# Kamino666/video_features

Hardware: NVIDIA H100
Metric: frames/sec CLIP-ViT-B/32 @224px (higher is better)
Workload: dtype f16

## Files before the change

video_features_b200/csrc/common.cuh:

```cuda
#pragma once
#include <cuda.h>
#include <cuda_runtime.h>
#include <cuda_fp16.h>
#include <stdint.h>

namespace vf {

__device__ __forceinline__ uint32_t smem_u32(const void* p) {
    return static_cast<uint32_t>(__cvta_generic_to_shared(p));
}

__device__ __forceinline__ void mbar_init(uint64_t* bar, uint32_t count) {
    asm volatile("mbarrier.init.shared::cta.b64 [%0], %1;" ::"r"(smem_u32(bar)), "r"(count));
}
__device__ __forceinline__ void fence_mbar_init() {
    asm volatile("fence.mbarrier_init.release.cluster;" ::: "memory");
}
__device__ __forceinline__ void mbar_expect_tx(uint64_t* bar, uint32_t bytes) {
    asm volatile("mbarrier.arrive.expect_tx.shared::cta.b64 _, [%0], %1;" ::"r"(smem_u32(bar)), "r"(bytes)
                 : "memory");
}
__device__ __forceinline__ void mbar_arrive(uint64_t* bar) {
    asm volatile("mbarrier.arrive.shared::cta.b64 _, [%0];" ::"r"(smem_u32(bar)) : "memory");
}
__device__ __forceinline__ void mbar_wait(uint64_t* bar, uint32_t parity) {
    asm volatile(
        "{\n"
        ".reg .pred P1;\n"
        "LAB_WAIT:\n"
        "mbarrier.try_wait.parity.shared::cta.b64 P1, [%0], %1;\n"
        "@P1 bra DONE;\n"
        "bra LAB_WAIT;\n"
        "DONE:\n"
        "}" ::"r"(smem_u32(bar)),
        "r"(parity)
        : "memory");
}

__device__ __forceinline__ void tma_prefetch_desc(const CUtensorMap* tm) {
    asm volatile("prefetch.tensormap [%0];" ::"l"(reinterpret_cast<uint64_t>(tm)) : "memory");
}
__device__ __forceinline__ void tma_load_2d(void* smem_dst, const CUtensorMap* tm, uint64_t* bar, int c0, int c1) {
    asm volatile(
        "cp.async.bulk.tensor.2d.shared::cluster.global.mbarrier::complete_tx::bytes [%0], [%1, {%3, %4}], [%2];" ::"r"(
            smem_u32(smem_dst)),
        "l"(reinterpret_cast<uint64_t>(tm)), "r"(smem_u32(bar)), "r"(c0), "r"(c1)
        : "memory");
}
__device__ __forceinline__ void tma_load_4d(void* smem_dst, const CUtensorMap* tm, uint64_t* bar, int c0, int c1,
                                            int c2, int c3) {
    asm volatile(
        "cp.async.bulk.tensor.4d.shared::cluster.global.mbarrier::complete_tx::bytes [%0], [%1, {%3, %4, %5, %6}], "
        "[%2];" ::"r"(smem_u32(smem_dst)),
        "l"(reinterpret_cast<uint64_t>(tm)), "r"(smem_u32(bar)), "r"(c0), "r"(c1), "r"(c2), "r"(c3)
        : "memory");
}
__device__ __forceinline__ void tma_load_5d(void* smem_dst, const CUtensorMap* tm, uint64_t* bar, int c0, int c1,
                                            int c2, int c3, int c4) {
    asm volatile(
        "cp.async.bulk.tensor.5d.shared::cluster.global.mbarrier::complete_tx::bytes [%0], [%1, {%3, %4, %5, %6, "
        "%7}], [%2];" ::"r"(smem_u32(smem_dst)),
        "l"(reinterpret_cast<uint64_t>(tm)), "r"(smem_u32(bar)), "r"(c0), "r"(c1), "r"(c2), "r"(c3), "r"(c4)
        : "memory");
}

__device__ __forceinline__ void tma_store_2d(const CUtensorMap* tm, const void* smem_src, int c0, int c1) {
    asm volatile("cp.async.bulk.tensor.2d.global.shared::cta.bulk_group [%0, {%2, %3}], [%1];" ::"l"(
                     reinterpret_cast<uint64_t>(tm)),
                 "r"(smem_u32(smem_src)), "r"(c0), "r"(c1)
                 : "memory");
}
__device__ __forceinline__ void tma_reduce_add_2d(const CUtensorMap* tm, const void* smem_src, int c0, int c1) {
    asm volatile("cp.reduce.async.bulk.tensor.2d.global.shared::cta.add.tile.bulk_group [%0, {%2, %3}], [%1];" ::"l"(
                     reinterpret_cast<uint64_t>(tm)),
                 "r"(smem_u32(smem_src)), "r"(c0), "r"(c1)
                 : "memory");
}
__device__ __forceinline__ void red_add_f32x4(float* gptr, float4 v) {
    asm volatile("red.global.add.v4.f32 [%0], {%1, %2, %3, %4};" ::"l"(gptr), "f"(v.x), "f"(v.y), "f"(v.z), "f"(v.w) : "memory");
}
__device__ __forceinline__ void bulk_commit() { asm volatile("cp.async.bulk.commit_group;" ::: "memory"); }
template <int N>
__device__ __forceinline__ void bulk_wait_read() {
    asm volatile("cp.async.bulk.wait_group.read %0;" ::"n"(N) : "memory");
}
template <int N>
__device__ __forceinline__ void bulk_wait() {
    asm volatile("cp.async.bulk.wait_group %0;" ::"n"(N) : "memory");
}
__device__ __forceinline__ void st_shared_b32(uint32_t addr, uint32_t v) {
    asm volatile("st.shared.b32 [%0], %1;" ::"r"(addr), "r"(v) : "memory");
}
__device__ __forceinline__ void st_shared_v2_f32(uint32_t addr, float x, float y) {
    asm volatile("st.shared.v2.f32 [%0], {%1, %2};" ::"r"(addr), "f"(x), "f"(y) : "memory");
}
__device__ __forceinline__ void fence_proxy_async() { asm volatile("fence.proxy.async.shared::cta;" ::: "memory"); }
__device__ __forceinline__ void named_bar_sync(uint32_t id, uint32_t nthreads) {
    asm volatile("bar.sync %0, %1;" ::"r"(id), "r"(nthreads) : "memory");
}
__device__ __forceinline__ void named_bar_arrive(uint32_t id, uint32_t nthreads) {
    asm volatile("bar.arrive %0, %1;" ::"r"(id), "r"(nthreads) : "memory");
}
template <uint32_t N>
__device__ __forceinline__ void setmaxnreg_dec() {
    asm volatile("setmaxnreg.dec.sync.aligned.u32 %0;" ::"n"(N));
}
template <uint32_t N>
__device__ __forceinline__ void setmaxnreg_inc() {
    asm volatile("setmaxnreg.inc.sync.aligned.u32 %0;" ::"n"(N));
}

__device__ __forceinline__ uint64_t wgmma_desc_sw128(const void* smem_tile) {
    uint64_t d = 0;
    d |= static_cast<uint64_t>((smem_u32(smem_tile) & 0x3FFFF) >> 4);
    d |= static_cast<uint64_t>(1) << 16;
    d |= static_cast<uint64_t>(1024 >> 4) << 32;
    d |= static_cast<uint64_t>(1) << 62;
    return d;
}
__device__ __forceinline__ void wgmma_fence() { asm volatile("wgmma.fence.sync.aligned;" ::: "memory"); }
__device__ __forceinline__ void wgmma_commit() { asm volatile("wgmma.commit_group.sync.aligned;" ::: "memory"); }
template <int N>
__device__ __forceinline__ void wgmma_wait() {
    asm volatile("wgmma.wait_group.sync.aligned %0;" ::"n"(N) : "memory");
}
template <int R>
__device__ __forceinline__ void wgmma_fence_regs(float* d) {
#pragma unroll
    for (int i = 0; i < R; ++i) asm volatile("" : "+f"(d[i])::"memory");
}

__device__ __forceinline__ float warp_sum(float v) {
#pragma unroll
    for (int o = 16; o > 0; o >>= 1) v += __shfl_xor_sync(0xffffffffu, v, o);
    return v;
}
__device__ __forceinline__ float warp_max(float v) {
#pragma unroll
    for (int o = 16; o > 0; o >>= 1) v = fmaxf(v, __shfl_xor_sync(0xffffffffu, v, o));
    return v;
}
__device__ __forceinline__ uint32_t pack_half2(float a, float b) {
    __half2 h = __floats2half2_rn(a, b);
    return *reinterpret_cast<uint32_t*>(&h);
}

}
```

video_features_b200/csrc/gemm.cu:

```cuda
#include "gemm_kernel.cuh"

namespace vf {

extern template int launch_bn<1, false, true>(GEMM_LAUNCH_ARGS);
extern template int launch_bn<1, true, true>(GEMM_LAUNCH_ARGS);
extern template int launch_bn<1, false, false>(GEMM_LAUNCH_ARGS);
extern template int launch_bn<1, true, false>(GEMM_LAUNCH_ARGS);
extern template int launch_bn<2, false, false>(GEMM_LAUNCH_ARGS);
extern template int launch_bn<2, true, false>(GEMM_LAUNCH_ARGS);

namespace {

typedef CUresult (*EncodeTiledFn)(CUtensorMap*, CUtensorMapDataType, cuuint32_t, void*, const cuuint64_t*,
                                  const cuuint64_t*, const cuuint32_t*, const cuuint32_t*, CUtensorMapInterleave,
                                  CUtensorMapSwizzle, CUtensorMapL2promotion, CUtensorMapFloatOOBfill);

EncodeTiledFn get_encode_tiled() {
    static EncodeTiledFn fn = nullptr;
    if (fn) return fn;
    void* p = nullptr;
    cudaDriverEntryPointQueryResult q;
    if (cudaGetDriverEntryPoint("cuTensorMapEncodeTiled", &p, cudaEnableDefault, &q) != cudaSuccess ||
        q != cudaDriverEntryPointSuccess)
        return nullptr;
    fn = reinterpret_cast<EncodeTiledFn>(p);
    return fn;
}

}

int device_sm_count() {
    static std::atomic<int> sms[64];
    int dev = 0;
    if (cudaGetDevice(&dev) != cudaSuccess || dev < 0 || dev >= 64) return 132;
    int v = sms[dev].load(std::memory_order_relaxed);
    if (v == 0) {
        if (cudaDeviceGetAttribute(&v, cudaDevAttrMultiProcessorCount, dev) != cudaSuccess || v <= 0) v = 132;
        sms[dev].store(v, std::memory_order_relaxed);
    }
    return v;
}

int make_tmap_2d(CUtensorMap* out, const void* base, int elem_bytes, uint64_t rows, uint64_t cols,
                 uint64_t row_pitch_bytes, uint32_t box_rows, uint32_t box_cols) {
    EncodeTiledFn enc = get_encode_tiled();
    if (!enc) return fail(VF_ERR_CUDA, "cuTensorMapEncodeTiled entry point unavailable (no CUDA driver?)");
    if ((reinterpret_cast<uintptr_t>(base) & 15) || (row_pitch_bytes & 15))
        return fail(VF_ERR_INVALID, "TMA operand must be 16-byte aligned with a 16-byte multiple row pitch");
    if (box_cols * uint32_t(elem_bytes) != 128) return fail(VF_ERR_INVALID, "TMA box rows must be 128 bytes");
    const CUtensorMapDataType dt = elem_bytes == 2 ? CU_TENSOR_MAP_DATA_TYPE_FLOAT16 : CU_TENSOR_MAP_DATA_TYPE_FLOAT32;
    cuuint64_t dims[2] = {cols, rows};
    cuuint64_t strides[1] = {row_pitch_bytes};
    cuuint32_t box[2] = {box_cols, box_rows};
    cuuint32_t estr[2] = {1, 1};
    CUresult r = enc(out, dt, 2, const_cast<void*>(base), dims, strides, box, estr, CU_TENSOR_MAP_INTERLEAVE_NONE,
                     CU_TENSOR_MAP_SWIZZLE_128B, CU_TENSOR_MAP_L2_PROMOTION_L2_256B, CU_TENSOR_MAP_FLOAT_OOB_FILL_NONE);
    if (r != CUDA_SUCCESS) return fail(VF_ERR_CUDA, "cuTensorMapEncodeTiled failed with CUresult %d", int(r));
    return VF_OK;
}

struct GemmProf {
    bool on = false;
    std::vector<cudaEvent_t> ev;
    size_t used = 0;
    double flops = 0.0;
};
static thread_local GemmProf g_prof;

template <bool PP>
static int run_gemm_launch(const CUtensorMap& tmA, const CUtensorMap& tmB, const CUtensorMap& tmD,
                           const CUtensorMap& tmD2, int bn, const GemmEpi& ep, int M, int N, const ConvGeom& cg,
                           cudaStream_t stream) {
    const bool split = ep.split_off > 0 && !ep.out_f32;
    if constexpr (!PP) {
        if (cg.nsplit == 2)
            return split ? launch_bn<2, true, PP>(tmA, tmB, tmD, tmD2, bn, ep, M, N, cg, stream)
                         : launch_bn<2, false, PP>(tmA, tmB, tmD, tmD2, bn, ep, M, N, cg, stream);
    }
    return split ? launch_bn<1, true, PP>(tmA, tmB, tmD, tmD2, bn, ep, M, N, cg, stream)
                 : launch_bn<1, false, PP>(tmA, tmB, tmD, tmD2, bn, ep, M, N, cg, stream);
}

static int run_gemm(const CUtensorMap& tmA, bool pp, const __half* B, int ldb, int64_t Ktot, int M, int N,
                    const ConvGeom& cg, const GemmEpi& ep, cudaStream_t stream) {
    if (!ep.out) return fail(VF_ERR_INVALID, "gemm: null output");
    if (reinterpret_cast<uintptr_t>(ep.out) & 15) return fail(VF_ERR_INVALID, "gemm: output must be 16-byte aligned");
    if (ep.accumulate && !ep.out_f32) return fail(VF_ERR_INVALID, "gemm: accumulate needs fp32 output");
    if (N % 8) return fail(VF_ERR_INVALID, "gemm: N=%d must be a multiple of 8", N);
    if (ep.act < VF_ACT_NONE || ep.act > VF_ACT_LEAKY) return fail(VF_ERR_INVALID, "gemm: unknown activation %d", ep.act);
    if (ep.out_f32 ? (ep.ldo % 4) : (ep.ldo % 8)) return fail(VF_ERR_INVALID, "gemm: ldo breaks 16-byte rows");
    if (ep.split_off && (ep.out_f32 || ep.split_off < N || ep.split_off % 8))
        return fail(VF_ERR_INVALID, "gemm: split output needs fp16 out and split_off >= N, multiple of 8");
    const int bm = tile_rows(pp);
    const int64_t num_m = (M + bm - 1) / bm, sms = device_sm_count();
    int bn = 256;
    int64_t best = INT64_MAX;
    for (int cand : {256, 192, 128, 64}) {
        const int64_t cost = (num_m * ((N + cand - 1) / cand) + sms - 1) / sms * cand;
        if (cost < best) { best = cost; bn = cand; }
    }
    CUtensorMap tmB, tmD, tmD2;
    VF_TRY(make_tmap_2d(&tmB, B, 2, uint64_t(N), uint64_t(Ktot), uint64_t(ldb) * 2, uint32_t(bn), BK));
    const int eb = ep.out_f32 ? 4 : 2;
    VF_TRY(make_tmap_2d(&tmD, ep.out, eb, uint64_t(M), uint64_t(N), uint64_t(ep.ldo) * eb, EPI_ROWS, 128 / eb));
    if (ep.split_off)
        VF_TRY(make_tmap_2d(&tmD2, static_cast<__half*>(ep.out) + ep.split_off, eb, uint64_t(M), uint64_t(N),
                            uint64_t(ep.ldo) * eb, EPI_ROWS, 128 / eb));
    else
        tmD2 = tmD;
    auto launch = [&] {
        return pp ? run_gemm_launch<true>(tmA, tmB, tmD, tmD2, bn, ep, M, N, cg, stream)
                  : run_gemm_launch<false>(tmA, tmB, tmD, tmD2, bn, ep, M, N, cg, stream);
    };
    if (!g_prof.on) return launch();
    if (g_prof.used + 2 > g_prof.ev.size())
        for (int i = 0; i < 2; ++i) {
            cudaEvent_t e;
            VF_CUDA(cudaEventCreate(&e));
            g_prof.ev.push_back(e);
        }
    VF_CUDA(cudaEventRecord(g_prof.ev[g_prof.used], stream));
    const int st = launch();
    VF_CUDA(cudaEventRecord(g_prof.ev[g_prof.used + 1], stream));
    g_prof.used += 2;
    double kexec = double(Ktot);
    if (cg.nsplit == 2 && cg.lo_mask) {
        const int kpt = (cg.k_per_tap + BK - 1) / BK;
        int skipped = 0;
        for (int kk = 0; kk < kpt && kk < 64; ++kk) skipped += int((cg.lo_mask >> kk) & 1ull);
        kexec -= double(cg.ntaps) * skipped * BK;
    }
    g_prof.flops += 2.0 * double(M) * double(N) * kexec;
    return st;
}

bool gemm_profile_on() { return g_prof.on; }
int gemm_profile(int enable) {
    g_prof.on = enable != 0;
    return VF_OK;
}
int gemm_profile_read(double* ms, int64_t* launches, double* flops) {
    VF_CUDA(cudaDeviceSynchronize());
    double t = 0.0;
    for (size_t i = 0; i + 1 < g_prof.used; i += 2) {
        float x = 0.f;
        VF_CUDA(cudaEventElapsedTime(&x, g_prof.ev[i], g_prof.ev[i + 1]));
        t += x;
    }
    if (ms) *ms = t;
    if (launches) *launches = int64_t(g_prof.used / 2);
    if (flops) *flops = g_prof.flops;
    g_prof.used = 0;
    g_prof.flops = 0.0;
    return VF_OK;
}

int gemm_f16(const __half* A, int lda, const __half* B, int ldb, int M, int N, int K, const GemmEpi& ep,
             cudaStream_t stream) {
    if (M <= 0 || N <= 0 || K <= 0) return fail(VF_ERR_INVALID, "gemm: empty problem %dx%dx%d", M, N, K);
    if (K % 8 || lda % 8 || ldb % 8) return fail(VF_ERR_INVALID, "gemm: K/lda/ldb must be multiples of 8");
    ConvGeom cg;
    memset(&cg, 0, sizeof(cg));
    cg.ntaps = 1;
    cg.k_per_tap = K;
    cg.nsplit = 1;
    CUtensorMap tmA;
    VF_TRY(make_tmap_2d(&tmA, A, 2, uint64_t(M), uint64_t(K), uint64_t(lda) * 2, tile_rows(true), BK));
    return run_gemm(tmA, true, B, ldb, K, M, N, cg, ep, stream);
}

int conv_gemm_f16(const __half* X, int C, int64_t P, const __half* Wt, int N, const ConvGeom& g, const GemmEpi& ep,
                  cudaStream_t stream) {
    if (P <= 0 || P > 0x7fffffff || N <= 0 || C <= 0) return fail(VF_ERR_INVALID, "conv_gemm: bad size");
    if (C % 8) return fail(VF_ERR_INVALID, "conv_gemm: C=%d must be a multiple of 8", C);
    if (g.ntaps < 1 || g.ntaps > 64 || g.k_per_tap < 8 || g.k_per_tap % 8)
        return fail(VF_ERR_INVALID, "conv_gemm: bad tap geometry (%d taps x %d)", g.ntaps, g.k_per_tap);
    if (g.nsplit != 1 && g.nsplit != 2) return fail(VF_ERR_INVALID, "conv_gemm: nsplit must be 1 or 2");
    const int kpt = (g.k_per_tap + BK - 1) / BK;
    if (g.lo_mask && (kpt > 64 || (kpt < 64 && (g.lo_mask >> kpt) != 0)))
        return fail(VF_ERR_INVALID, "conv_gemm: lo_mask 0x%llx names K blocks beyond the %d of a tap", g.lo_mask, kpt);
    if (g.mask && (g.Tp < 1 || g.Hp < 1 || g.Wp < 1 || g.row0 < 0))
        return fail(VF_ERR_INVALID, "conv_gemm: bad mask volume %dx%dx%d, row0 %d", g.Tp, g.Hp, g.Wp, g.row0);
    CUtensorMap tmA;
    VF_TRY(make_tmap_2d(&tmA, X, 2, uint64_t(P), uint64_t(g.k_per_tap), uint64_t(C) * 2, tile_rows(false), BK));
    const int64_t Ktot = int64_t(g.ntaps) * g.k_per_tap * g.nsplit;
    if (Ktot % 8) return fail(VF_ERR_INVALID, "conv_gemm: K must be a multiple of 8");
    return run_gemm(tmA, false, Wt, int(Ktot), Ktot, int(P), N, g, ep, stream);
}

}
```

video_features_b200/csrc/gemm_inst_pp.cu:

```cuda
#include "gemm_kernel.cuh"

namespace vf {
template int launch_bn<1, false, true>(GEMM_LAUNCH_ARGS);
template int launch_bn<1, true, true>(GEMM_LAUNCH_ARGS);
}
```

video_features_b200/csrc/gemm_kernel.cuh:

```cuda
#pragma once
#include <stdarg.h>
#include <stdlib.h>
#include <string.h>

#include <atomic>
#include <vector>

#include "common.cuh"
#include "internal.h"
#include "wgmma.cuh"

namespace vf {

namespace {

constexpr int BK = 64;
constexpr int THREADS = 384;
constexpr uint32_t PRODUCER_REGS = 40, CONSUMER_REGS = 232;
constexpr int EPI_ROWS = 64;
constexpr uint32_t STG_BYTES = EPI_ROWS * 128;
constexpr uint32_t STAGING_BYTES = 2 * 2 * STG_BYTES;
constexpr uint32_t SMEM_LIMIT = 227 * 1024;
constexpr uint32_t MAX_STAGES = 8;
constexpr uint32_t RING_BUDGET = SMEM_LIMIT - STAGING_BYTES - 2 * MAX_STAGES * 8 - 1024;

template <int BN, int NSPLIT, bool PP>
struct GemmCfg {
    static constexpr int BM = PP ? 64 : 128;
    static constexpr uint32_t A_BYTES = BM * BK * 2;
    static constexpr uint32_t B_TILE = BN * BK * 2;
    static constexpr uint32_t B_BYTES = NSPLIT * B_TILE;
    static constexpr uint32_t STAGE_BYTES = A_BYTES + B_BYTES;
    static constexpr int STAGES = RING_BUDGET / STAGE_BYTES > MAX_STAGES ? MAX_STAGES : int(RING_BUDGET / STAGE_BYTES);
    static constexpr uint32_t BAR_BYTES = 2 * STAGES * 8;
    static constexpr uint32_t SMEM_BYTES = STAGES * STAGE_BYTES + STAGING_BYTES + BAR_BYTES + 1024;
    static_assert(STAGES >= 2, "at least two pipeline stages");
    static_assert(SMEM_BYTES <= SMEM_LIMIT, "shared memory budget");
    static_assert(A_BYTES % 1024 == 0 && B_TILE % 1024 == 0, "swizzle-128B tiles must stay 1024-byte aligned");
};

constexpr int tile_rows(bool pp) { return pp ? GemmCfg<64, 1, true>::BM : GemmCfg<64, 1, false>::BM; }

template <int ACT>
__device__ __forceinline__ float apply_act(float v) {
    if (ACT == VF_ACT_QUICKGELU) {
        return __fdividef(v, 1.0f + __expf(-1.702f * v));
    } else if (ACT == VF_ACT_RELU) {
        return fmaxf(v, 0.0f);
    } else if (ACT == VF_ACT_SIGMOID) {
        return __fdividef(1.0f, 1.0f + __expf(-v));
    } else if (ACT == VF_ACT_TANH) {
        return 1.0f - __fdividef(2.0f, 1.0f + __expf(2.0f * v));
    } else if (ACT == VF_ACT_LEAKY) {
        return v > 0.0f ? v : __fmul_rn(v, 0.1f);
    }
    return v;
}

template <int BN, int NSPLIT, bool SPLIT, bool PP, int ACT>
__global__ void __launch_bounds__(THREADS, 1)
gemm_f16_kernel(const __grid_constant__ CUtensorMap tmA, const __grid_constant__ CUtensorMap tmB,
                const __grid_constant__ CUtensorMap tmD, const __grid_constant__ CUtensorMap tmD2, const GemmEpi ep,
                const int M, const int N, const __grid_constant__ ConvGeom cg) {
    using Cfg = GemmCfg<BN, NSPLIT, PP>;
    static_assert(PP ? NSPLIT == 1 : true, "split weights run in the conv mode only");
    constexpr int STAGES = Cfg::STAGES;
    constexpr int BM = Cfg::BM;
    extern __shared__ uint8_t smem_raw[];
    uint8_t* smem = reinterpret_cast<uint8_t*>((reinterpret_cast<uintptr_t>(smem_raw) + 1023) & ~uintptr_t(1023));
    uint8_t* sA = smem;
    uint8_t* sB = smem + STAGES * Cfg::A_BYTES;
    uint8_t* sD = smem + STAGES * Cfg::STAGE_BYTES;
    uint64_t* full = reinterpret_cast<uint64_t*>(sD + STAGING_BYTES);
    uint64_t* empty = full + STAGES;

    const int warp = threadIdx.x >> 5;
    const int lane = threadIdx.x & 31;
    const int num_m = (M + BM - 1) / BM;
    const int num_n = (N + BN - 1) / BN;
    const int num_tiles = num_m * num_n;
    auto tile_m0 = [&](int tile) { return (PP ? tile / num_n : tile % num_m) * BM; };
    auto tile_n0 = [&](int tile) { return (PP ? tile % num_n : tile / num_m) * BN; };
    const int cta_tiles = (num_tiles - 1 - int(blockIdx.x)) / int(gridDim.x) + 1;
    const int kpt = (cg.k_per_tap + BK - 1) / BK;
    const int num_k = cg.ntaps * kpt;

    if (threadIdx.x == 0) {
        tma_prefetch_desc(&tmA);
        tma_prefetch_desc(&tmB);
        tma_prefetch_desc(&tmD);
        if (SPLIT) tma_prefetch_desc(&tmD2);
        for (int i = 0; i < STAGES; ++i) {
            mbar_init(&full[i], 1);
            mbar_init(&empty[i], PP ? 4 : 8);
        }
        fence_mbar_init();
    }
    __syncthreads();

    if (warp < 4) {
        setmaxnreg_dec<PRODUCER_REGS>();
        if (warp == 0 && lane == 0) {
            int stage = 0;
            uint32_t phase = 0;
            for (int i = 0; i < cta_tiles; ++i) {
                const int tile = blockIdx.x + i * gridDim.x;
                const int m0 = tile_m0(tile), n0 = tile_n0(tile);
                for (int tap = 0; tap < cg.ntaps; ++tap) {
                    const int arow = m0 + cg.tap_off[tap];
                    const int bcol = tap * cg.k_per_tap;
                    for (int kk = 0; kk < kpt; ++kk) {
                        mbar_wait(&empty[stage], phase ^ 1);
                        const bool lo_blk = NSPLIT == 2 && ((cg.lo_mask >> kk) & 1ull);
                        mbar_expect_tx(&full[stage], Cfg::A_BYTES + (lo_blk ? Cfg::B_TILE : Cfg::B_BYTES));
                        tma_load_2d(sA + stage * Cfg::A_BYTES, &tmA, &full[stage], kk * BK, arow);
                        tma_load_2d(sB + stage * Cfg::B_BYTES, &tmB, &full[stage], bcol + kk * BK, n0);
                        if (NSPLIT == 2 && !lo_blk)
                            tma_load_2d(sB + stage * Cfg::B_BYTES + Cfg::B_TILE, &tmB, &full[stage],
                                        cg.ntaps * cg.k_per_tap + bcol + kk * BK, n0);
                        if (++stage == STAGES) { stage = 0; phase ^= 1; }
                    }
                }
            }
        }
        return;
    }

    setmaxnreg_inc<CONSUMER_REGS>();
    const int wg = (warp >> 2) - 1;
    const int wq = warp & 3;
    constexpr int R = BN / 2;
    float acc[R];
    const bool issuer = (threadIdx.x & 127) == 0;
    uint32_t buf = 0;
    auto wg_sync = [&] {
        if (wg == 0) named_bar_sync(1, 128);
        else named_bar_sync(2, 128);
    };
    auto store_subtile = [&](int col, int row) {
        fence_proxy_async();
        if (issuer) bulk_wait_read<0>();
        wg_sync();
        if (issuer) {
            const uint8_t* src = sD + (wg * 2 + buf) * STG_BYTES;
            if (ep.accumulate) tma_reduce_add_2d(&tmD, src, col, row);
            else tma_store_2d(&tmD, src, col, row);
            bulk_commit();
        }
        buf ^= 1;
    };
    auto wait_turn = [&] {
        if (wg == 0) named_bar_sync(3, 256);
        else named_bar_sync(4, 256);
    };
    auto pass_turn = [&] {
        if (wg == 0) named_bar_arrive(4, 256);
        else named_bar_arrive(3, 256);
    };
    for (int i = PP ? wg : 0; i < cta_tiles; i += PP ? 2 : 1) {
        const int tile = blockIdx.x + i * gridDim.x;
        const int m0 = tile_m0(tile) + (PP ? 0 : wg * 64), n0 = tile_n0(tile);
        const uint64_t first = uint64_t(i) * uint64_t(num_k);
        int stage = int(first % STAGES);
        uint32_t phase = uint32_t(first / STAGES) & 1u;
        if (PP && i > 0) wait_turn();
        int prev = -1;
        for (int kb = 0, kk = 0; kb < num_k; ++kb) {
            mbar_wait(&full[stage], phase);
            const uint64_t adesc = wgmma_desc_sw128(sA + stage * Cfg::A_BYTES + (PP ? 0 : wg * (64 * 128)));
            const uint64_t bdesc = wgmma_desc_sw128(sB + stage * Cfg::B_BYTES);
            const bool lo_blk = NSPLIT == 2 && ((cg.lo_mask >> kk) & 1ull);
            wgmma_fence_regs<R>(acc);
            wgmma_fence();
#pragma unroll
            for (int k = 0; k < BK / 16; ++k) {
                Wgmma<BN>::mma(acc, adesc + 2 * k, bdesc + 2 * k, (kb | k) != 0 ? 1u : 0u);
                if (NSPLIT == 2 && !lo_blk) Wgmma<BN>::mma(acc, adesc + 2 * k, bdesc + (Cfg::B_TILE >> 4) + 2 * k, 1u);
            }
            wgmma_commit();
            wgmma_wait<1>();
            wgmma_fence_regs<R>(acc);
            if (prev >= 0) {
                __syncwarp();
                if (lane == 0) mbar_arrive(&empty[prev]);
            }
            prev = stage;
            if (++stage == STAGES) { stage = 0; phase ^= 1; }
            if (++kk == kpt) kk = 0;
        }
        if (PP && i + 1 < cta_tiles) pass_turn();
        float2 sc[8], bi[8];
        auto load_sb = [&](int s) {
#pragma unroll
            for (int c = 0; c < 8; ++c) {
                const int n = min(n0 + 64 * s + 8 * c + 2 * (lane & 3), N - 2);
                sc[c] = ep.scale ? __ldg(reinterpret_cast<const float2*>(ep.scale + n)) : make_float2(1.f, 1.f);
                bi[c] = ep.bias ? __ldg(reinterpret_cast<const float2*>(ep.bias + n)) : make_float2(-0.f, -0.f);
            }
        };
        load_sb(0);
        wgmma_wait<0>();
        wgmma_fence_regs<R>(acc);
        __syncwarp();
        if (lane == 0) mbar_arrive(&empty[prev]);

        bool keep[2] = {true, true};
        if (cg.mask) {
#pragma unroll
            for (int h = 0; h < 2; ++h) {
                const int mm = m0 + wq * 16 + (lane >> 2) + 8 * h - cg.row0;
                const int w = mm % cg.Wp, r1 = mm / cg.Wp;
                const int hh = r1 % cg.Hp, r2 = r1 / cg.Hp;
                const int tt = r2 % cg.Tp;
                keep[h] = (mm >= 0) && (w >= cg.w0) && (w < cg.w1) && (hh >= cg.h0) && (hh < cg.h1) && (tt >= cg.t0) && (tt < cg.t1);
            }
        }
        const int row = m0;
        const uint32_t stg = smem_u32(sD) + wg * 2 * STG_BYTES + (wq * 16 + (lane >> 2)) * 128;
        const int swz = lane >> 2;
#pragma unroll
        for (int s = 0; s < BN / 64; ++s) {
            if (n0 + 64 * s >= N) break;
#pragma unroll
            for (int c = 0; c < 8; ++c)
#pragma unroll
                for (int h = 0; h < 2; ++h) {
                    const int j = 8 * s + c;
                    float v0 = __fadd_rn(__fmul_rn(acc[4 * j + 2 * h], sc[c].x), bi[c].x);
                    float v1 = __fadd_rn(__fmul_rn(acc[4 * j + 2 * h + 1], sc[c].y), bi[c].y);
                    v0 = apply_act<ACT>(v0);
                    v1 = apply_act<ACT>(v1);
                    acc[4 * j + 2 * h] = keep[h] ? v0 : 0.f;
                    acc[4 * j + 2 * h + 1] = keep[h] ? v1 : 0.f;
                }
            if (s + 1 < BN / 64) load_sb(s + 1);
            if (SPLIT) {
                if (issuer) bulk_wait_read<0>();
                wg_sync();
#pragma unroll
                for (int c = 0; c < 8; ++c)
#pragma unroll
                    for (int h = 0; h < 2; ++h) {
                        const int j = 8 * s + c;
                        const float v0 = acc[4 * j + 2 * h], v1 = acc[4 * j + 2 * h + 1];
                        const __half2 hi = __floats2half2_rn(v0, v1);
                        const uint32_t off = h * 8 * 128 + ((c ^ swz) << 4) + 4 * (lane & 3);
                        st_shared_b32(stg + off, *reinterpret_cast<const uint32_t*>(&hi));
                        st_shared_b32(stg + STG_BYTES + off, pack_half2(v0 - __low2float(hi), v1 - __high2float(hi)));
                    }
                fence_proxy_async();
                wg_sync();
                if (issuer) {
                    tma_store_2d(&tmD, sD + wg * 2 * STG_BYTES, n0 + 64 * s, row);
                    tma_store_2d(&tmD2, sD + (wg * 2 + 1) * STG_BYTES, n0 + 64 * s, row);
                    bulk_commit();
                }
            } else if (ep.out_f32) {
#pragma unroll
                for (int q = 0; q < 2; ++q) {
                    if (q == 1 && n0 + 64 * s + 32 >= N) break;
                    const uint32_t d = stg + buf * STG_BYTES;
#pragma unroll
                    for (int c = 0; c < 4; ++c) {
                        const int j = 8 * s + 4 * q + c;
                        const int chunk = 2 * c + ((lane & 3) >> 1);
#pragma unroll
                        for (int h = 0; h < 2; ++h)
                            st_shared_v2_f32(d + h * 8 * 128 + ((chunk ^ swz) << 4) + 8 * (lane & 1), acc[4 * j + 2 * h],
                                             acc[4 * j + 2 * h + 1]);
                    }
                    store_subtile(n0 + 64 * s + 32 * q, row);
                }
            } else {
                const uint32_t d = stg + buf * STG_BYTES;
#pragma unroll
                for (int c = 0; c < 8; ++c)
#pragma unroll
                    for (int h = 0; h < 2; ++h) {
                        const int j = 8 * s + c;
                        st_shared_b32(d + h * 8 * 128 + ((c ^ swz) << 4) + 4 * (lane & 3),
                                      pack_half2(acc[4 * j + 2 * h], acc[4 * j + 2 * h + 1]));
                    }
                store_subtile(n0 + 64 * s, row);
            }
        }
    }
    if (issuer) bulk_wait<0>();
}

template <int BN, int NSPLIT, bool SPLIT, bool PP, int ACT>
int launch_gemm(const CUtensorMap& tmA, const CUtensorMap& tmB, const CUtensorMap& tmD, const CUtensorMap& tmD2,
                const GemmEpi& ep, int M, int N, const ConvGeom& cg, cudaStream_t stream) {
    using Cfg = GemmCfg<BN, NSPLIT, PP>;
    static std::atomic<bool> attr_set[64];
    int dev = 0;
    VF_CUDA(cudaGetDevice(&dev));
    if (dev < 0 || dev >= 64 || !attr_set[dev].load(std::memory_order_acquire)) {
        VF_CUDA(cudaFuncSetAttribute(gemm_f16_kernel<BN, NSPLIT, SPLIT, PP, ACT>,
                                     cudaFuncAttributeMaxDynamicSharedMemorySize, Cfg::SMEM_BYTES));
        if (dev >= 0 && dev < 64) attr_set[dev].store(true, std::memory_order_release);
    }
    const int tiles = ((M + Cfg::BM - 1) / Cfg::BM) * ((N + BN - 1) / BN);
    const int sms = device_sm_count();
    const int grid = tiles < sms ? tiles : sms;
    gemm_f16_kernel<BN, NSPLIT, SPLIT, PP, ACT><<<grid, THREADS, Cfg::SMEM_BYTES, stream>>>(tmA, tmB, tmD, tmD2, ep, M,
                                                                                            N, cg);
    VF_CUDA(cudaGetLastError());
    return VF_OK;
}

template <int BN, int NSPLIT, bool SPLIT, bool PP>
int launch_act(const CUtensorMap& tmA, const CUtensorMap& tmB, const CUtensorMap& tmD, const CUtensorMap& tmD2,
               const GemmEpi& ep, int M, int N, const ConvGeom& cg, cudaStream_t stream) {
    switch (ep.act) {
        case VF_ACT_QUICKGELU:
            return launch_gemm<BN, NSPLIT, SPLIT, PP, VF_ACT_QUICKGELU>(tmA, tmB, tmD, tmD2, ep, M, N, cg, stream);
        case VF_ACT_RELU:
            return launch_gemm<BN, NSPLIT, SPLIT, PP, VF_ACT_RELU>(tmA, tmB, tmD, tmD2, ep, M, N, cg, stream);
        case VF_ACT_SIGMOID:
            return launch_gemm<BN, NSPLIT, SPLIT, PP, VF_ACT_SIGMOID>(tmA, tmB, tmD, tmD2, ep, M, N, cg, stream);
        case VF_ACT_TANH:
            return launch_gemm<BN, NSPLIT, SPLIT, PP, VF_ACT_TANH>(tmA, tmB, tmD, tmD2, ep, M, N, cg, stream);
        case VF_ACT_LEAKY:
            if constexpr (NSPLIT == 2 && !PP)
                return launch_gemm<BN, NSPLIT, SPLIT, PP, VF_ACT_LEAKY>(tmA, tmB, tmD, tmD2, ep, M, N, cg, stream);
            else
                return fail(VF_ERR_INVALID, "gemm: LeakyReLU is built for split-weight convolutions (nsplit = 2) only");
        default:
            return launch_gemm<BN, NSPLIT, SPLIT, PP, VF_ACT_NONE>(tmA, tmB, tmD, tmD2, ep, M, N, cg, stream);
    }
}

}

#define GEMM_LAUNCH_ARGS                                                                                           \
    const CUtensorMap &tmA, const CUtensorMap &tmB, const CUtensorMap &tmD, const CUtensorMap &tmD2, int bn,       \
        const GemmEpi &ep, int M, int N, const ConvGeom &cg, cudaStream_t stream
template <int NSPLIT, bool SPLIT, bool PP>
int launch_bn(GEMM_LAUNCH_ARGS) {
    if (bn == 256) return launch_act<256, NSPLIT, SPLIT, PP>(tmA, tmB, tmD, tmD2, ep, M, N, cg, stream);
    if (bn == 192) return launch_act<192, NSPLIT, SPLIT, PP>(tmA, tmB, tmD, tmD2, ep, M, N, cg, stream);
    if (bn == 128) return launch_act<128, NSPLIT, SPLIT, PP>(tmA, tmB, tmD, tmD2, ep, M, N, cg, stream);
    return launch_act<64, NSPLIT, SPLIT, PP>(tmA, tmB, tmD, tmD2, ep, M, N, cg, stream);
}

}
```

Before: 46070.

## Use 2-CTA clusters with TMA multicast of B tiles in ping-pong GEMM

Launches the ping-pong GEMM kernel as 2-CTA clusters. The two CTAs handle adjacent M tiles and share the same N tile, and each loads half of the B tile and multicasts it to both CTAs. Empty barriers are released across the cluster, and the number of resident clusters is queried through the occupancy API to size the grid and choose BN. The goal is to halve L2 traffic for B, at the cost of cluster scheduling constraints, cross-CTA barrier coupling and possible loss of SM coverage if clusters do not pack evenly.

```diff
diff --git a/video_features_b200/csrc/common.cuh b/video_features_b200/csrc/common.cuh
--- a/video_features_b200/csrc/common.cuh
+++ b/video_features_b200/csrc/common.cuh
@@ -37,6 +37,25 @@
         : "memory");
 }
 
+__device__ __forceinline__ uint32_t cluster_ctarank() {
+    uint32_t r;
+    asm volatile("mov.u32 %0, %%cluster_ctarank;" : "=r"(r));
+    return r;
+}
+__device__ __forceinline__ void cluster_sync() {
+    __syncwarp();
+    asm volatile("barrier.cluster.arrive.release.aligned;\n\tbarrier.cluster.wait.acquire.aligned;" ::: "memory");
+}
+__device__ __forceinline__ void mbar_arrive_cluster(uint64_t* bar, uint32_t cta) {
+    asm volatile(
+        "{\n\t.reg .b32 ra;\n\t"
+        "mapa.shared::cluster.u32 ra, %0, %1;\n\t"
+        "mbarrier.arrive.shared::cluster.b64 _, [ra];\n\t"
+        "}" ::"r"(smem_u32(bar)),
+        "r"(cta)
+        : "memory");
+}
+
 __device__ __forceinline__ void tma_prefetch_desc(const CUtensorMap* tm) {
     asm volatile("prefetch.tensormap [%0];" ::"l"(reinterpret_cast<uint64_t>(tm)) : "memory");
 }
@@ -45,6 +64,14 @@
         "cp.async.bulk.tensor.2d.shared::cluster.global.mbarrier::complete_tx::bytes [%0], [%1, {%3, %4}], [%2];" ::"r"(
             smem_u32(smem_dst)),
         "l"(reinterpret_cast<uint64_t>(tm)), "r"(smem_u32(bar)), "r"(c0), "r"(c1)
+        : "memory");
+}
+__device__ __forceinline__ void tma_load_2d_multicast(void* smem_dst, const CUtensorMap* tm, uint64_t* bar, int c0,
+                                                      int c1, uint16_t ctamask) {
+    asm volatile(
+        "cp.async.bulk.tensor.2d.shared::cluster.global.mbarrier::complete_tx::bytes.multicast::cluster [%0], [%1, {%3, "
+        "%4}], [%2], %5;" ::"r"(smem_u32(smem_dst)),
+        "l"(reinterpret_cast<uint64_t>(tm)), "r"(smem_u32(bar)), "r"(c0), "r"(c1), "h"(ctamask)
         : "memory");
 }
 __device__ __forceinline__ void tma_load_4d(void* smem_dst, const CUtensorMap* tm, uint64_t* bar, int c0, int c1,
diff --git a/video_features_b200/csrc/gemm.cu b/video_features_b200/csrc/gemm.cu
--- a/video_features_b200/csrc/gemm.cu
+++ b/video_features_b200/csrc/gemm.cu
@@ -92,15 +92,22 @@
     if (ep.split_off && (ep.out_f32 || ep.split_off < N || ep.split_off % 8))
         return fail(VF_ERR_INVALID, "gemm: split output needs fp16 out and split_off >= N, multiple of 8");
     const int bm = tile_rows(pp);
-    const int64_t num_m = (M + bm - 1) / bm, sms = device_sm_count();
+    const int64_t num_m = (M + bm - 1) / bm;
+    int64_t units = device_sm_count();
+    if (pp) {
+        int clusters = 0;
+        VF_TRY(gemm_pp_clusters(&clusters));
+        units = clusters;
+    }
+    const int64_t rows = pp ? (num_m + 1) / 2 : num_m;
     int bn = 256;
     int64_t best = INT64_MAX;
     for (int cand : {256, 192, 128, 64}) {
-        const int64_t cost = (num_m * ((N + cand - 1) / cand) + sms - 1) / sms * cand;
+        const int64_t cost = (rows * ((N + cand - 1) / cand) + units - 1) / units * cand;
         if (cost < best) { best = cost; bn = cand; }
     }
     CUtensorMap tmB, tmD, tmD2;
-    VF_TRY(make_tmap_2d(&tmB, B, 2, uint64_t(N), uint64_t(Ktot), uint64_t(ldb) * 2, uint32_t(bn), BK));
+    VF_TRY(make_tmap_2d(&tmB, B, 2, uint64_t(N), uint64_t(Ktot), uint64_t(ldb) * 2, uint32_t(pp ? bn / 2 : bn), BK));
     const int eb = ep.out_f32 ? 4 : 2;
     VF_TRY(make_tmap_2d(&tmD, ep.out, eb, uint64_t(M), uint64_t(N), uint64_t(ep.ldo) * eb, EPI_ROWS, 128 / eb));
     if (ep.split_off)
diff --git a/video_features_b200/csrc/gemm_inst_pp.cu b/video_features_b200/csrc/gemm_inst_pp.cu
--- a/video_features_b200/csrc/gemm_inst_pp.cu
+++ b/video_features_b200/csrc/gemm_inst_pp.cu
@@ -3,4 +3,25 @@
 namespace vf {
 template int launch_bn<1, false, true>(GEMM_LAUNCH_ARGS);
 template int launch_bn<1, true, true>(GEMM_LAUNCH_ARGS);
+
+int gemm_pp_clusters(int* clusters) {
+    static std::atomic<int> cached[64];
+    int dev = 0;
+    VF_CUDA(cudaGetDevice(&dev));
+    const bool keep = dev >= 0 && dev < 64;
+    int n = keep ? cached[dev].load(std::memory_order_relaxed) : 0;
+    if (n == 0) {
+        using Cfg = GemmCfg<64, 1, true>;
+        const auto kernel = gemm_f16_kernel<64, 1, false, true, VF_ACT_NONE>;
+        VF_CUDA(cudaFuncSetAttribute(kernel, cudaFuncAttributeMaxDynamicSharedMemorySize, Cfg::SMEM_BYTES));
+        cudaLaunchConfig_t cfg = {};
+        cudaLaunchAttribute attr;
+        pp_cluster_config(&cfg, &attr, 2, Cfg::SMEM_BYTES, 0);
+        VF_CUDA(cudaOccupancyMaxActiveClusters(&n, kernel, &cfg));
+        if (n < 1) return fail(VF_ERR_CUDA, "gemm: no 2-CTA cluster of the GEMM kernel fits on device %d", dev);
+        if (keep) cached[dev].store(n, std::memory_order_relaxed);
+    }
+    *clusters = n;
+    return VF_OK;
 }
+}
diff --git a/video_features_b200/csrc/gemm_kernel.cuh b/video_features_b200/csrc/gemm_kernel.cuh
--- a/video_features_b200/csrc/gemm_kernel.cuh
+++ b/video_features_b200/csrc/gemm_kernel.cuh
@@ -11,6 +11,8 @@
 #include "wgmma.cuh"
 
 namespace vf {
+
+int gemm_pp_clusters(int* clusters);
 
 namespace {
 
@@ -36,6 +38,7 @@
     static constexpr uint32_t SMEM_BYTES = STAGES * STAGE_BYTES + STAGING_BYTES + BAR_BYTES + 1024;
     static_assert(STAGES >= 2, "at least two pipeline stages");
     static_assert(SMEM_BYTES <= SMEM_LIMIT, "shared memory budget");
+    static_assert(!PP || 2 * SMEM_BYTES > 228 * 1024, "ping-pong instantiations share one resident-cluster count");
     static_assert(A_BYTES % 1024 == 0 && B_TILE % 1024 == 0, "swizzle-128B tiles must stay 1024-byte aligned");
 };
 
@@ -78,10 +81,13 @@
     const int lane = threadIdx.x & 31;
     const int num_m = (M + BM - 1) / BM;
     const int num_n = (N + BN - 1) / BN;
-    const int num_tiles = num_m * num_n;
-    auto tile_m0 = [&](int tile) { return (PP ? tile / num_n : tile % num_m) * BM; };
+    const int rank = PP ? int(cluster_ctarank()) : 0;
+    const int unit = PP ? int(blockIdx.x) / 2 : int(blockIdx.x);
+    const int units = PP ? int(gridDim.x) / 2 : int(gridDim.x);
+    const int num_tiles = (PP ? (num_m + 1) / 2 : num_m) * num_n;
+    auto tile_m0 = [&](int tile) { return (PP ? 2 * (tile / num_n) + rank : tile % num_m) * BM; };
     auto tile_n0 = [&](int tile) { return (PP ? tile % num_n : tile / num_m) * BN; };
-    const int cta_tiles = (num_tiles - 1 - int(blockIdx.x)) / int(gridDim.x) + 1;
+    const int cta_tiles = (num_tiles - 1 - unit) / units + 1;
     const int kpt = (cg.k_per_tap + BK - 1) / BK;
     const int num_k = cg.ntaps * kpt;
 
@@ -92,11 +98,12 @@
         if (SPLIT) tma_prefetch_desc(&tmD2);
         for (int i = 0; i < STAGES; ++i) {
             mbar_init(&full[i], 1);
-            mbar_init(&empty[i], PP ? 4 : 8);
+            mbar_init(&empty[i], 8);
         }
         fence_mbar_init();
     }
-    __syncthreads();
+    if (PP) cluster_sync();
+    else __syncthreads();
 
     if (warp < 4) {
         setmaxnreg_dec<PRODUCER_REGS>();
@@ -104,7 +111,7 @@
             int stage = 0;
             uint32_t phase = 0;
             for (int i = 0; i < cta_tiles; ++i) {
-                const int tile = blockIdx.x + i * gridDim.x;
+                const int tile = unit + i * units;
                 const int m0 = tile_m0(tile), n0 = tile_n0(tile);
                 for (int tap = 0; tap < cg.ntaps; ++tap) {
                     const int arow = m0 + cg.tap_off[tap];
@@ -114,7 +121,11 @@
                         const bool lo_blk = NSPLIT == 2 && ((cg.lo_mask >> kk) & 1ull);
                         mbar_expect_tx(&full[stage], Cfg::A_BYTES + (lo_blk ? Cfg::B_TILE : Cfg::B_BYTES));
                         tma_load_2d(sA + stage * Cfg::A_BYTES, &tmA, &full[stage], kk * BK, arow);
-                        tma_load_2d(sB + stage * Cfg::B_BYTES, &tmB, &full[stage], bcol + kk * BK, n0);
+                        if (PP)
+                            tma_load_2d_multicast(sB + stage * Cfg::B_BYTES + rank * (BN / 2) * 128, &tmB, &full[stage],
+                                                  bcol + kk * BK, n0 + rank * (BN / 2), 0b11);
+                        else
+                            tma_load_2d(sB + stage * Cfg::B_BYTES, &tmB, &full[stage], bcol + kk * BK, n0);
                         if (NSPLIT == 2 && !lo_blk)
                             tma_load_2d(sB + stage * Cfg::B_BYTES + Cfg::B_TILE, &tmB, &full[stage],
                                         cg.ntaps * cg.k_per_tap + bcol + kk * BK, n0);
@@ -123,6 +134,7 @@
                 }
             }
         }
+        if (PP) cluster_sync();
         return;
     }
 
@@ -157,8 +169,16 @@
         if (wg == 0) named_bar_arrive(4, 256);
         else named_bar_arrive(3, 256);
     };
+    auto release = [&](int s) {
+        __syncwarp();
+        if (PP) {
+            if (lane < 2) mbar_arrive_cluster(&empty[s], uint32_t(lane));
+        } else if (lane == 0) {
+            mbar_arrive(&empty[s]);
+        }
+    };
     for (int i = PP ? wg : 0; i < cta_tiles; i += PP ? 2 : 1) {
-        const int tile = blockIdx.x + i * gridDim.x;
+        const int tile = unit + i * units;
         const int m0 = tile_m0(tile) + (PP ? 0 : wg * 64), n0 = tile_n0(tile);
         const uint64_t first = uint64_t(i) * uint64_t(num_k);
         int stage = int(first % STAGES);
@@ -180,10 +200,7 @@
             wgmma_commit();
             wgmma_wait<1>();
             wgmma_fence_regs<R>(acc);
-            if (prev >= 0) {
-                __syncwarp();
-                if (lane == 0) mbar_arrive(&empty[prev]);
-            }
+            if (prev >= 0) release(prev);
             prev = stage;
             if (++stage == STAGES) { stage = 0; phase ^= 1; }
             if (++kk == kpt) kk = 0;
@@ -201,8 +218,7 @@
         load_sb(0);
         wgmma_wait<0>();
         wgmma_fence_regs<R>(acc);
-        __syncwarp();
-        if (lane == 0) mbar_arrive(&empty[prev]);
+        release(prev);
 
         bool keep[2] = {true, true};
         if (cg.mask) {
@@ -286,6 +302,21 @@
         }
     }
     if (issuer) bulk_wait<0>();
+    if (PP) cluster_sync();
+}
+
+inline void pp_cluster_config(cudaLaunchConfig_t* cfg, cudaLaunchAttribute* attr, int grid, uint32_t smem,
+                              cudaStream_t stream) {
+    attr->id = cudaLaunchAttributeClusterDimension;
+    attr->val.clusterDim.x = 2;
+    attr->val.clusterDim.y = 1;
+    attr->val.clusterDim.z = 1;
+    cfg->gridDim = dim3(grid);
+    cfg->blockDim = dim3(THREADS);
+    cfg->dynamicSmemBytes = smem;
+    cfg->stream = stream;
+    cfg->attrs = attr;
+    cfg->numAttrs = 1;
 }
 
 template <int BN, int NSPLIT, bool SPLIT, bool PP, int ACT>
@@ -293,18 +324,29 @@
                 const GemmEpi& ep, int M, int N, const ConvGeom& cg, cudaStream_t stream) {
     using Cfg = GemmCfg<BN, NSPLIT, PP>;
     static std::atomic<bool> attr_set[64];
+    const auto kernel = gemm_f16_kernel<BN, NSPLIT, SPLIT, PP, ACT>;
     int dev = 0;
     VF_CUDA(cudaGetDevice(&dev));
-    if (dev < 0 || dev >= 64 || !attr_set[dev].load(std::memory_order_acquire)) {
-        VF_CUDA(cudaFuncSetAttribute(gemm_f16_kernel<BN, NSPLIT, SPLIT, PP, ACT>,
-                                     cudaFuncAttributeMaxDynamicSharedMemorySize, Cfg::SMEM_BYTES));
-        if (dev >= 0 && dev < 64) attr_set[dev].store(true, std::memory_order_release);
-    }
-    const int tiles = ((M + Cfg::BM - 1) / Cfg::BM) * ((N + BN - 1) / BN);
-    const int sms = device_sm_count();
-    const int grid = tiles < sms ? tiles : sms;
-    gemm_f16_kernel<BN, NSPLIT, SPLIT, PP, ACT><<<grid, THREADS, Cfg::SMEM_BYTES, stream>>>(tmA, tmB, tmD, tmD2, ep, M,
-                                                                                            N, cg);
+    const bool cached = dev >= 0 && dev < 64;
+    if (!cached || !attr_set[dev].load(std::memory_order_acquire)) {
+        VF_CUDA(cudaFuncSetAttribute(kernel, cudaFuncAttributeMaxDynamicSharedMemorySize, Cfg::SMEM_BYTES));
+        if (cached) attr_set[dev].store(true, std::memory_order_release);
+    }
+    const int num_m = (M + Cfg::BM - 1) / Cfg::BM, num_n = (N + BN - 1) / BN;
+    if constexpr (!PP) {
+        const int tiles = num_m * num_n;
+        const int sms = device_sm_count();
+        const int grid = tiles < sms ? tiles : sms;
+        kernel<<<grid, THREADS, Cfg::SMEM_BYTES, stream>>>(tmA, tmB, tmD, tmD2, ep, M, N, cg);
+    } else {
+        int clusters = 0;
+        VF_TRY(gemm_pp_clusters(&clusters));
+        const int tiles = (num_m + 1) / 2 * num_n;
+        cudaLaunchConfig_t cfg = {};
+        cudaLaunchAttribute attr;
+        pp_cluster_config(&cfg, &attr, 2 * (tiles < clusters ? tiles : clusters), Cfg::SMEM_BYTES, stream);
+        VF_CUDA(cudaLaunchKernelEx(&cfg, kernel, tmA, tmB, tmD, tmD2, ep, M, N, cg));
+    }
     VF_CUDA(cudaGetLastError());
     return VF_OK;
 }
```

After: 46880, median of 6. +1.8%, better.
